# harvardinformatics/IMCoalHMM

Hardware: AMD Instinct MI355X
Metric: alignment columns/sec (forward pass), 20-state isolation HMM (higher is better)
Workload: dtype f64

## Files before the change

imcoalhmm_amd/csrc/imcoal_fwd.hip:

```cpp
#include <hip/hip_runtime.h>

#include <algorithm>
#include <array>
#include <cerrno>
#include <climits>
#include <cmath>
#include <cstdint>
#include <cstdio>
#include <cstdlib>
#include <cstring>
#include <list>
#include <atomic>
#include <chrono>
#include <map>
#include <set>
#include <memory>
#include <mutex>
#include <condition_variable>
#include <string>
#include <vector>

#include <sys/stat.h>
#include <unistd.h>

// ... 5 lines not shown
#include "kernels_zip2.hpp"
#include "kernels_zip3.hpp"
#include "kernels_zip4.hpp"
#include "pair_dict.hpp"
#include "kernels_encode.hpp"
#include "kernels_train.hpp"
#include "kernels_ingest.hpp"
#include "kernels_align.hpp"
#include "plan_host.hpp"
#include "planner_host.hpp"
#include "model_host.hpp"
#include "kernels_model.hpp"
#include "../../include/imcoal_model.h"
#include "obs_io.hpp"
#include "fasta_io.hpp"

static_assert(sizeof(imc::Desc4) == sizeof(int4) && alignof(imc::Desc4) == alignof(int4), "descriptor entries are uploaded as int4");

namespace {

thread_local std::string g_err;
std::mutex g_mu;
std::condition_variable g_cv;

int fail(int code, const std::string &msg)
{
    g_err = msg;
    return code;
}

#define HIP_TRY(expr)                                                                                   \
    do {                                                                                                \
        hipError_t _e = (expr);                                                                         \
        if (_e != hipSuccess)                                                                           \
            return fail(_e == hipErrorOutOfMemory ? IMC_ERR_OOM : IMC_ERR_HIP,                          \
                        std::string(#expr) + ": " + hipGetErrorString(_e));                             \
    } while (0)

using imc::HYBRID_MAX_ALPHABET;
using imc::LDS_BUDGET;
using imc::Z2GRAN;
using imc::round_up;

constexpr size_t STAGE_KERNEL_MAX_BYTES = 1u << 20;

hipError_t dev_alloc(void **p, size_t bytes);
void dev_free(void *p);

struct DictDev : imc::TrainedDict {
    uint16_t *d_left = nullptr, *d_right = nullptr;
    uint16_t *d_order = nullptr;
    uint64_t trained_on = 0;
    pid_t pid = 0;
    DictDev(imc::TrainedDict t, uint64_t columns) : imc::TrainedDict(std::move(t)), trained_on(columns) {}
    ~DictDev()
    {
        if (pid == getpid()) { dev_free(d_left); dev_free(d_right); dev_free(d_order); }
    }
};

struct Ev3 { hipEvent_t a, b, c; };

struct Ctx {
    pid_t pid = 0;
    int device = -1;
    bool ready = false;
    hipStream_t stream = nullptr;
    int cus = 256;
    uint64_t next_obs_id = 1, next_dict_id = 1;
    size_t seg_override = 0;
    int compression = 1;
    int kernel_pref = 0;
    bool profile = false;
    bool rank1_handoff = true;
    int blocked_variant = 4;
    int wide_blocked = -1;
    int z4_stream = -1;
    bool table_pairs = true;
    int table_triples = -1;
    bool table_split = true;
    int table_split_max = -1;
    bool xcd_affine = true;
    int fuse_tail = 1;
    bool fuse_head = true;
    bool pack_table = true;
    int device_encode = -1;
    bool guard = false;
    bool use_graphs = false;
    std::vector<Ev3> events;
    std::map<int, std::shared_ptr<DictDev>> dicts;
    uint64_t last_plan[8] = {0, 0, 0, 0, 0, 0, 0, 0};
    uint64_t last_ingest[4] = {0, 0, 0, 0};
    int device_ingest = -1;
    int device_train = -1;
    uint64_t last_training[4] = {0, 0, 0, 0};
    uint64_t r1_checked = 0, r1_collapsed = 0;
    std::string last_kernels;
    std::vector<const void *> lds_opted;
} g;

void drop_plans();
void drop_plans_using(imc_obs *const *obs, size_t n);
void wait_all_idle(std::unique_lock<std::mutex> &lk);
void model_release();

int ensure_ctx()
{
    const pid_t me = getpid();
    if (g.ready && g.pid == me) return IMC_OK;
    if (g.ready && g.pid != me)
        return fail(IMC_ERR_HIP, "libimcoal_fwd was initialised in the parent process before fork(): fork the chain "
                                 "processes before the first imc_* call of the parent, or use the spawn start method");
    int n = 0;
    if (hipGetDeviceCount(&n) != hipSuccess || n <= 0)
        return fail(IMC_ERR_NODEVICE, "no HIP device available (libimcoal_fwd has no CPU fallback)");
    if (g.device < 0) {
        int cur = 0;
        if (hipGetDevice(&cur) != hipSuccess) cur = 0;
        g.device = cur;
    }
    if (g.device >= n) return fail(IMC_ERR_NODEVICE, "requested device index out of range");
    HIP_TRY(hipSetDevice(g.device));
    hipDeviceProp_t prop;
    HIP_TRY(hipGetDeviceProperties(&prop, g.device));
    if (std::strncmp(prop.gcnArchName, "gfx950", 6) != 0)
        return fail(IMC_ERR_NODEVICE, std::string("device is ") + prop.gcnArchName + ", this library is built for gfx950 only");
    g.cus = prop.multiProcessorCount > 0 ? prop.multiProcessorCount : 256;
    HIP_TRY(hipStreamCreateWithFlags(&g.stream, hipStreamNonBlocking));
    g.use_graphs = std::getenv("IMC_GRAPH") != nullptr;
    if (const char *gd = std::getenv("IMC_GUARD")) g.guard = std::atoi(gd) != 0;
    if (const char *bv = std::getenv("IMC_BLOCKED")) { const int v = std::atoi(bv); if (v >= 2 && v <= 5) g.blocked_variant = v; }
    if (const char *r1 = std::getenv("IMC_RANK1")) g.rank1_handoff = std::atoi(r1) != 0;
    if (const char *pt = std::getenv("IMC_PACK_TABLE")) g.pack_table = std::atoi(pt) != 0;
    if (const char *tp = std::getenv("IMC_TABLE_PAIRS")) g.table_pairs = std::atoi(tp) != 0;
    if (const char *fh = std::getenv("IMC_FUSE_HEAD")) g.fuse_head = std::atoi(fh) != 0;
    if (const char *ts = std::getenv("IMC_TABLE_SPLIT")) g.table_split = std::atoi(ts) != 0;
    if (const char *tm = std::getenv("IMC_TABLE_SPLIT_MAX")) g.table_split_max = std::max(0, std::atoi(tm));
    if (const char *tt = std::getenv("IMC_TABLE_TRIPLES")) g.table_triples = std::atoi(tt) != 0 ? 1 : 0;
    if (const char *ft = std::getenv("IMC_FUSE_TAIL")) g.fuse_tail = std::max(0, std::min(2, std::atoi(ft)));
    if (const char *xa = std::getenv("IMC_XCD_AFFINE")) g.xcd_affine = std::atoi(xa) != 0;
    if (const char *wb = std::getenv("IMC_WIDE_BLOCKED")) { const int v = std::atoi(wb); if (v >= -1 && v <= 1) g.wide_blocked = v; }
    if (g.device_encode < 0) {
        const char *de = std::getenv("IMC_DEVICE_ENCODE");
        g.device_encode = de && std::atoi(de) == 1 ? 1 : 0;
    }
    if (const char *zs = std::getenv("IMC_Z4_STREAM")) { const int v = std::atoi(zs); if (v >= -1 && v <= 1) g.z4_stream = v; }
    g.pid = me;
    g.ready = true;
    return IMC_OK;
}

struct GuardRec { hipDeviceptr_t va; size_t va_size; hipMemGenericAllocationHandle_t handle; hipDeviceptr_t map; size_t map_size; };
std::map<void *, GuardRec> &g_guard = *new std::map<void *, GuardRec>();

hipError_t dev_alloc(void **p, size_t bytes)
{
    bytes = std::max<size_t>(bytes, 16);
    if (!g.guard) return hipMalloc(p, bytes);
    hipMemAllocationProp prop{};
    prop.type = hipMemAllocationTypePinned;
    prop.location.type = hipMemLocationTypeDevice;
    prop.location.id = g.device;
    size_t gran = 0;
    hipError_t e = hipMemGetAllocationGranularity(&gran, &prop, hipMemAllocationGranularityMinimum);
    if (e != hipSuccess || gran == 0) return e != hipSuccess ? e : hipErrorUnknown;
    GuardRec r{};
    r.map_size = (bytes + gran - 1) / gran * gran;
    r.va_size = r.map_size + 2 * gran;
    e = hipMemAddressReserve(&r.va, r.va_size, gran, nullptr, 0);
    if (e != hipSuccess) return e;
    e = hipMemCreate(&r.handle, r.map_size, &prop, 0);
    if (e != hipSuccess) { (void)hipMemAddressFree(r.va, r.va_size); return e; }
    r.map = (hipDeviceptr_t)((char *)r.va + gran);
    e = hipMemMap(r.map, r.map_size, 0, r.handle, 0);
    if (e == hipSuccess) {
        hipMemAccessDesc ad{};
        ad.location = prop.location;
        ad.flags = hipMemAccessFlagsProtReadWrite;
        e = hipMemSetAccess(r.map, r.map_size, &ad, 1);
        if (e != hipSuccess) (void)hipMemUnmap(r.map, r.map_size);
    }
    if (e != hipSuccess) { (void)hipMemRelease(r.handle); (void)hipMemAddressFree(r.va, r.va_size); return e; }
    void *user = (char *)r.map + (r.map_size - (bytes + 15) / 16 * 16);
    g_guard[user] = r;
    *p = user;
    return hipSuccess;
}

void dev_free(void *p)
{
    if (!p) return;
    auto it = g_guard.find(p);
    if (it == g_guard.end()) { (void)hipFree(p); return; }
    (void)hipDeviceSynchronize();
    (void)hipMemUnmap(it->second.map, it->second.map_size);
    (void)hipMemRelease(it->second.handle);
    g_guard.erase(it);
}

template <class T>
class DevBuf {
    T *p_ = nullptr;

public:
    DevBuf() = default;
    DevBuf(const DevBuf &) = delete;
    DevBuf &operator=(const DevBuf &) = delete;
    DevBuf(DevBuf &&o) noexcept : p_(o.p_) { o.p_ = nullptr; }
    DevBuf &operator=(DevBuf &&o) noexcept
    {
        if (this != &o) { reset(); p_ = o.p_; o.p_ = nullptr; }
        return *this;
    }
    ~DevBuf() { reset(); }
    hipError_t alloc(size_t bytes)
    {
        reset();
        return dev_alloc((void **)&p_, bytes);
    }
    void reset()
    {
        dev_free(p_);
        p_ = nullptr;
// ... 1192 lines not shown
}

int recompress_alphabet(int nsym, std::vector<imc_obs *> &obs, bool on_device)
{
    std::sort(obs.begin(), obs.end(), [](const imc_obs *x, const imc_obs *y) { return x->id < y->id; });
    obs.erase(std::unique(obs.begin(), obs.end()), obs.end());
    const bool wide_raw = nsym > imc::kByteAlphabet;
    const size_t unit = wide_raw ? sizeof(imc::tok_t) : 1;
    PhaseTimer tm;
    size_t total = 0;
    for (imc_obs *o : obs) total += o->L;
    if (total < imc::TrainLimits().train_min) return IMC_OK;
    const size_t share = imc::recompress_share(obs.size(), wide_raw);
    std::vector<std::vector<uint8_t>> raw(obs.size());
    bool train_on_device = false;
    size_t copied = 0;
    {
        std::lock_guard<std::mutex> lk(g_mu);
        train_on_device = device_train_mode() == 1;
        bool same = obs[0]->dict != nullptr;
        for (imc_obs *o : obs) same = same && o->dict == obs[0]->dict;
        if (same && obs[0]->dict->trained_on >= total) return IMC_OK;
        HIP_TRY(hipSetDevice(g.device));
        for (size_t k = 0; k < obs.size() && !(train_on_device && on_device); ++k) {
            raw[k].resize((on_device ? std::min(obs[k]->L, share) : obs[k]->L) * unit);
            HIP_TRY(hipMemcpy(raw[k].data(), obs[k]->d_sym, raw[k].size(), hipMemcpyDeviceToHost));
            copied += raw[k].size();
        }
    }
    std::vector<uint8_t> sample;
    if (!train_on_device) sample = imc::recompress_sample(raw, share, unit);
    tm.mark();
    std::shared_ptr<DictDev> nd;
    if (train_on_device) {
        std::vector<TrainPiece> pieces;
        size_t sample_len = 0;
        for (imc_obs *o : obs) {
            pieces.push_back({o->d_sym, (int)unit, std::min(o->L, share)});
            sample_len += pieces.back().n;
        }
        std::lock_guard<std::mutex> lk(g_mu);
        HIP_TRY(hipSetDevice(g.device));
        if (int rc = device_train(pieces.data(), pieces.size(), nsym, sample_len, total, &nd)) return rc;
    } else {
        imc::TrainStats st;
        nd = make_dictionary(symbols_in(sample, wide_raw), nsym, total, &st);
        std::vector<uint8_t>().swap(sample);
        std::lock_guard<std::mutex> lk(g_mu);
        note_training(0, st);
    }
    tm.mark();
    std::vector<imc::EncodedLevels> enc(obs.size());
    const bool zipped = nd->dict.alphabet > nsym;
    if (zipped && !on_device)
        for (size_t k = 0; k < obs.size(); ++k) {
            const HostSymbols sym = symbols_in(raw[k], wide_raw);
            imc::encode_levels(nd->dict, sym.bytes, sym.wide, obs[k]->L, enc[k]);
            std::vector<uint8_t>().swap(raw[k]);
        }
    tm.mark();
    std::unique_lock<std::mutex> lk(g_mu);
    wait_all_idle(lk);
    HIP_TRY(hipSetDevice(g.device));
    HIP_TRY(hipDeviceSynchronize());
    drop_plans_using(obs.data(), obs.size());
    if (!zipped) return IMC_OK;
    if (int rc = publish_dictionary(nsym, nd)) return rc;
    if (on_device) {
        for (imc_obs *o : obs) release_tokens(o);
        if (int rc = device_encode(nd, obs.data(), obs.size())) return rc;
    } else
        for (size_t k = 0; k < obs.size(); ++k) {
            release_tokens(obs[k]);
            if (int rc = install_encoding(obs[k], nd, enc[k])) return rc;
        }
    tm.mark();
    if (PhaseTimer::enabled())
        std::fprintf(stderr, "[imc host] recompress %zu chunks, %zu columns: copy back %.1f ms, train %.1f ms, encode %.1f ms, install %.1f ms (%s encoder, %s trainer, %zu symbol bytes to the host)\n",
                     obs.size(), total, tm.ms(0), tm.ms(1), tm.ms(2), tm.ms(3), on_device ? "device" : "host", train_on_device ? "device" : "host", copied);
    return IMC_OK;
}


using ChainFn = void (*)(const ChainDesc *, int, const uint32_t *, uint32_t, uint32_t, const double *, const int *,
                         const int *, uint32_t, double *, int *, double *, int);

struct KernelChoice : imc::KernelFacts {
    void (*plain)(PropArgs) = nullptr;
    void (*zip)(PropArgs) = nullptr;
    ChainFn chain = nullptr;
    void (*big_table_raw)(BigArgs) = nullptr;
    void (*big_table_level)(BigArgs, const uint16_t *, int) = nullptr;
    void (*big_prop)(BigArgs, const BigBlock *) = nullptr;
    int big_prop_waves = 0;
    void (*big_vec)(BigArgs, const BigBlock *, int, int) = nullptr;
    void (*big_vec_tail)(BigArgs, const BigBlock *, int, int) = nullptr;
    int big_vec_waves = 0;
    void (*zip2)(BigArgs) = nullptr;
    void (*zip3)(BigArgs) = nullptr;
    void (*zip4)(BigArgs) = nullptr;
    void (*zip4w)(BigArgs) = nullptr;
    void (*zip4s)(BigArgs) = nullptr, (*zip4sw)(BigArgs) = nullptr;
    void (*zip4_raw)(BigArgs) = nullptr;
    void (*zip4_level)(BigArgs, int, int) = nullptr;
    void (*zip4_level2)(BigArgs, const int4 *, int, int, const double *) = nullptr;
    void (*zip4_level2_first)(BigArgs, const int4 *, int, int, const double *) = nullptr;
    void (*zip4_level2_split)(BigArgs, const int4 *, int, int, const double *) = nullptr;
    void (*zip4_level2_split_first)(BigArgs, const int4 *, int, int, const double *) = nullptr;
    void (*zip4_level3)(BigArgs, const int4 *, int, int, const double *) = nullptr;
    void (*zip4_level3_first)(BigArgs, const int4 *, int, int, const double *) = nullptr;
    size_t (*zip4_level3_lds)(size_t) = nullptr;
    bool chain_self_emax = false;
    void note_kernels()
    {
        has_zip2 = zip2 != nullptr; has_zip3 = zip3 != nullptr; has_zip4 = zip4 != nullptr; has_zip4s = zip4s != nullptr;
        has_level2 = zip4_level2 != nullptr;
    }
};

template <int R, int G, int MW>
KernelChoice make_kc()
{
    constexpr int NP = R * G;
    KernelChoice k;
    k.R = R; k.G = G; k.NP = NP; k.VPW = 64 / G; k.minw = MW;
    k.zwaves = ZWAVES;
    k.z4_waves = Z2WAVES;
    k.plain = k_propagate<R, G, MW>;
    k.zip = k_zpropagate<R, G>;
    k.zip_lds = &ZipGeom<R, G>::lds_bytes;
    k.chain = k_chain<NP, (NP <= 12 ? 6 : NP <= 24 ? 4 : NP <= 32 ? 3 : NP <= 64 ? 2 : 1)>;
    k.chain_self_emax = true;
    if constexpr (NP % 4 == 0 && NP <= 24) {
        k.zip2 = k_zpropagate2<NP / 4>;
        k.zip2_lds = &Zip2Geom<NP / 4>::lds_bytes;
        k.zip3 = k_zpropagate3<NP / 4>;
        k.zip3_lds = &Zip3Geom<NP / 4>::lds_bytes;
        k.tok_doubles = Zip3Geom<NP / 4>::TOK;
        if constexpr (NP <= 24) {
            k.zip4 = k_zpropagate4<NP / 4, false, true>;
            k.zip4w = k_zpropagate4<NP / 4, true, true>;
            k.zip4s = k_zpropagate4<NP / 4, false, false>;
            k.zip4sw = k_zpropagate4<NP / 4, true, false>;
            k.zip4_raw = k_z4_raw<NP / 4>;
            k.zip4_level = k_z4_level<NP / 4>;
            k.zip4_level2 = k_z4_level2<NP / 4, false>;
            k.zip4_level2_first = k_z4_level2<NP / 4, true>;
            k.zip4_level2_split = k_z4_level2<NP / 4, false, Z4_SPLIT_WAVES>;
            k.zip4_level2_split_first = k_z4_level2<NP / 4, true, Z4_SPLIT_WAVES_FIRST>;
            k.zip4_level3 = k_z4_level3<NP / 4, false>;
            k.zip4_level3_first = k_z4_level3<NP / 4, true>;
            k.zip4_level3_lds = &Z4L3Geom<NP / 4>::lds_bytes;
            k.zip4_lds = &Zip4Geom<NP / 4>::lds_bytes;
            k.zip4_max_hot = &Zip4Geom<NP / 4>::max_hot;
        }
    }
    if constexpr (NP == 28 || NP == 32) {
        k.tok_doubles = Zip3Geom<NP / 4>::TOK;
        k.zip4s = k_zpropagate4<NP / 4, false, false>;
        k.zip4sw = k_zpropagate4<NP / 4, true, false>;
        k.zip4_raw = k_z4_raw<NP / 4>;
        k.zip4_level = k_z4_level<NP / 4>;
        k.zip4_lds = &Zip4Geom<NP / 4>::lds_bytes;
        k.z4_waves = Zip4Shape<NP / 4>::WAVES;
        k.wide_blocked = true;
    }
    k.note_kernels();
    return k;
}

template <int NT, int NSLAB>
KernelChoice make_big()
{
    constexpr bool dealt = NT > 4 && NT % 4 != 0;
    KernelChoice k;
    k.G = NT; k.NP = 16 * NT;
    k.z4_waves = Z2WAVES;
    k.chain = k_chain<16 * NT, 0>;
    k.big_table_raw = k_big_table_raw<NT>;
    k.big_table_level = k_big_table_level<NT>;
    k.big_prop = k_big_propagate<NT, NSLAB>;
    if constexpr (dealt) k.big_prop = k_big_propagate_s<NT, NSLAB>;
    k.big_prop_waves = dealt ? BS_WAVES : NT;
    k.big_vec = k_big_vector<NT, false>;
    k.big_vec_tail = k_big_vector<NT, true>;
    k.big_vec_waves = BigVec<NT>::WAVES;
    k.big_nslab = NSLAB;
    k.big_lds = BigSlab<NT, NSLAB>::bytes;
    return k;
}

KernelChoice kChoices[] = {
    make_kc<4, 1, 2>(), make_kc<4, 2, 2>(), make_kc<4, 3, 2>(), make_kc<4, 4, 2>(), make_kc<4, 5, 2>(),
    make_kc<3, 8, 2>(), make_kc<2, 14, 2>(), make_kc<2, 16, 2>(), make_kc<2, 20, 1>(), make_kc<1, 48, 1>(),
    make_kc<1, 56, 1>(), make_kc<1, 64, 1>(),
    make_big<6, 1>(), make_big<7, 1>(), make_big<8, 2>(), make_big<9, 3>(), make_big<10, 2>(), make_big<12, 3>(), make_big<14, 7>(),
    make_big<16, 8>(),
};
constexpr int IMC_MAX_N = 256;

KernelChoice kMidChoices[] = {make_big<2, 1>(), make_big<3, 1>(), make_big<4, 1>()};

KernelChoice *choose_kernel(int N, bool prefer_gemm)
{
    if (prefer_gemm && N > 24 && N <= 64)
        for (auto &k : kMidChoices)
            if (k.NP >= N) return &k;
    for (auto &k : kChoices)
        if (k.NP >= N) return &k;
    return nullptr;
}


struct Group {
    using Kind = imc::GroupKind;
    Kind kind = Kind::ColumnVector;
    bool is_chain() const { return kind == Kind::GemmChain || kind == Kind::MatVecChain; }
    bool is_blocked() const { return kind == Kind::BlockedLds || kind == Kind::BlockedGlobal; }
    bool global_table() const { return kind == Kind::BlockedGlobal; }

    bool tokens = false;
    int level = -1, A = 0;
    std::shared_ptr<DictDev> dict;
    std::vector<int> chunks;
    uint32_t vec_begin = 0, n_vecs = 0;
    size_t seglen = 0;
    double model_us = 0.0, model_tab_us = 0.0;
    uint64_t vsteps = 0;
    uint64_t stream_len = 0;
    DevBuf<double> d_Ctab;
    DevBuf<int> d_cex;

    struct Chain {
        std::vector<uint32_t> seg_ids, seg_out;
        std::vector<BigBlock> big_blocks;
        DevBuf<BigBlock> d_big_blocks;
        std::vector<std::pair<int, int>> table_runs;
        DevBuf<double> d_Cpack;
        bool rank1 = false;
        std::vector<int> checkpoints;
        std::vector<BigBlock> tail_blocks;
        std::vector<std::pair<uint32_t, uint32_t>> r1_segs;
        DevBuf<BigBlock> d_tail_blocks;
        DevBuf<int> d_r1flag, d_r1at;
        DevBuf<double> d_r1u, d_r1alpha;
    } chain;

    struct Blocked {
        std::vector<Z2Block> blocks;
        DevBuf<Z2Block> d_blocks;
        DevBuf<uint16_t> d_tab_order;
        DevBuf<int> d_tab_lvl;
        std::vector<int> tab_lvl;
        int tab_nlvl = 0;
        DevBuf<int4> d_tab_desc;
        DevBuf<int4> d_tab_desc2;
        std::vector<std::pair<int, int>> tab2;
        DevBuf<int4> d_tab_desc3;
        std::vector<std::pair<int, int>> tab3;
        bool wide_tokens = false;
        bool stream_table = false;
// ... 170 lines not shown
        chunk_unit.assign(n_chunks + 1, 0);
        for (int f = 0; f < n_chunks; ++f) chunk_unit[f + 1] = chunk_unit[f] + (uint32_t)chunk_units[f].size();
        unit_vec0.assign(chunk_unit[n_chunks], 0);
        unit_first.assign(chunk_unit[n_chunks], 0);
        for (Group &gr : p->groups) {
            gr.vec_begin = (uint32_t)vecs.size();
            for (int f : gr.chunks) {
                gr.stream_len += gr.tokens ? chunks[f]->ntok[gr.level] : chunks[f]->L;
                for (size_t u = 0; u < chunk_units[f].size(); ++u) {
                    const uint32_t sid = chunk_units[f][u].first, ns = chunk_units[f][u].second;
                    const uint32_t uid = chunk_unit[f] + (uint32_t)u;
                    const bool fst = seg_first[sid] != 0;
                    unit_first[uid] = fst;
                    unit_vec0[uid] = (uint32_t)vecs.size();
                    const int nv = fst ? 1 : N;
                    for (int c = 0; c < nv; ++c) vecs.push_back(VecDesc{sid, (uint32_t)c});
                    if (gr.is_chain()) { gr.chain.seg_ids.push_back(sid); gr.chain.seg_out.push_back(unit_vec0[uid]); }
                    if (gr.is_blocked()) {
                        std::vector<Z2Block> &blocks = gr.blk.blocks;
                        const bool whole = mfma() && fst && ns == 1 && chunk_units[f].size() == 1;
                        if (whole && !blocks.empty() && blocks.back().first == 2 && blocks.back().n < (uint32_t)kc->z4_slots() &&
                            blocks.back().seg0 + blocks.back().n == sid && blocks.back().out_vec0 + blocks.back().n == unit_vec0[uid])
                            ++blocks.back().n;
                        else
                            blocks.push_back(Z2Block{sid, ns, unit_vec0[uid], whole ? 2u : fst ? 1u : 0u});
                    }
                    for (uint32_t q2 = 0; q2 < ns; ++q2)
                        gr.vsteps += (uint64_t)((seg_first[sid + q2] && !gr.is_blocked()) ? 1 : N) * segs[sid + q2].len;
                }
            }
            gr.n_vecs = (uint32_t)vecs.size() - gr.vec_begin;
        }
        if (p->groups.size() == 1 && p->groups[0].is_blocked() && mfma() && !op_mode && n_chunks > 0) {
            Group::Blocked &bl = p->groups[0].blk;
            bool ok = true;
            size_t most = 0;
            for (int f = 0; f < n_chunks; ++f) {
                ok = ok && !chunk_units[f].empty() && chunk_units[f].size() <= (size_t)kc->z4_slots();
                most = std::max(most, chunk_units[f].size());
            }
            if (ok) {
                for (int f : p->groups[0].chunks)
                    for (size_t u = 0; u < chunk_units[f].size(); ++u)
                        bl.tails.push_back(Z2Tail{(uint32_t)f, (uint32_t)u, (uint32_t)chunk_units[f].size(), 0u});
                bl.tail_stride = (int)most;
                if (bl.tails.size() != bl.blocks.size()) bl.tails.clear();
                else
                    for (Z2Block &bk : bl.blocks)
                        if (bk.first == 2) bk.first = 1;
            }
        }
        if (vecs.size() >= (size_t)UINT32_MAX / 2) return fail(IMC_ERR_ARG, "too many vectors in one call");
        p->n_segs = (uint32_t)segs.size();
        p->n_vecs = (uint32_t)vecs.size();
        p->pstride = round_up((size_t)kc->NP + (size_t)kc->NP * kc->NP + (size_t)S * kc->NP, 2);

        return IMC_OK;
    }

    void make_hierarchy()
    {
        hl.assign(1, HostLevel());
        hl[0].chunk_seg = chunk_unit; hl[0].vec0 = unit_vec0; hl[0].first = unit_first; hl[0].n_vecs = p->n_vecs;
        for (;;) {
            const HostLevel &cur = hl.back();
            uint32_t kmax = 0;
            for (int f = 0; f < n_chunks; ++f) kmax = std::max(kmax, cur.chunk_seg[f + 1] - cur.chunk_seg[f]);
            if (kmax <= 1 && hl.size() > 1) break;
            if (kmax == 0) break;
            const uint32_t gsz = kmax <= 16 ? kmax : std::max<uint32_t>(12, (uint32_t)std::ceil(std::cbrt((double)kmax)));
            p->chain_steps += gsz;
            HostLevel nx;
            nx.chunk_seg.assign(n_chunks + 1, 0);
            nx.n_vecs = 0;
            for (int f = 0; f < n_chunks; ++f) {
                nx.chunk_seg[f] = (uint32_t)nx.vec0.size();
                const uint32_t s0 = cur.chunk_seg[f], s1 = cur.chunk_seg[f + 1];
                for (uint32_t rb = s0; rb < s1; rb += gsz) {
                    const uint32_t re = std::min(rb + gsz, s1);
                    const bool fst = rb == s0 && !op_mode;
                    nx.vec0.push_back(nx.n_vecs);
                    nx.first.push_back(fst);
                    const int nvv = fst ? 1 : N;
                    for (int c = 0; c < nvv; ++c) nx.chains.push_back(ChainDesc{rb, re, (uint32_t)c, nx.n_vecs + c, fst ? 1u : 0u, 0u});
                    nx.n_vecs += nvv;
                }
            }
            nx.chunk_seg[n_chunks] = (uint32_t)nx.vec0.size();
            const bool done = kmax <= gsz;
            hl.push_back(std::move(nx));
            if (done) break;
        }
        final_vec.assign(std::max(n_chunks, 1), -1);
        bool all_from_chains = hl.size() > 1 && !op_mode && n_chunks > 0;
        for (int f = 0; f < n_chunks; ++f) {
            const HostLevel &last = hl.back();
            if (last.chunk_seg[f + 1] > last.chunk_seg[f]) final_vec[f] = (int32_t)last.vec0[last.chunk_seg[f]];
            else all_from_chains = false;
        }
        p->finish_fused = false;
        if (all_from_chains) {
            HostLevel &last = hl.back();
            std::vector<char> seen((size_t)n_chunks, 0);
            for (ChainDesc &cd : last.chains)
                for (int f = 0; f < n_chunks; ++f)
                    if (cd.first && final_vec[f] == (int32_t)cd.out_vec) { cd.chunk1 = (uint32_t)f + 1; seen[f] = 1; }
            p->finish_fused = std::all_of(seen.begin(), seen.end(), [](char c) { return c != 0; });
            if (!p->finish_fused)
                for (ChainDesc &cd : last.chains) cd.chunk1 = 0;
        }

    }

    int upload(Plan **out)
    {
        while (g_plans.size() >= MAX_PLANS) {
            auto victim = g_plans.end();
            for (auto it = g_plans.begin(); it != g_plans.end(); ++it)
                if (!(*it)->busy) victim = it;
            if (victim == g_plans.end()) break;
            g_plans.erase(victim);
        }

        Plan *q = p.get();
        DevUpload u;
        u.put(q->d_segs, segs);
        u.put(q->d_vecs, vecs);
        u.put(q->d_final_vec, final_vec);
        q->levels.resize(hl.size());
        for (size_t l = 0; l < hl.size(); ++l) {
            Level &lv = q->levels[l];
            lv.n_segs = (uint32_t)hl[l].vec0.size();
            lv.n_vecs = hl[l].n_vecs;
            lv.n_chains = (uint32_t)hl[l].chains.size();
            const size_t nv = std::max<size_t>(lv.n_vecs, 1), ns = std::max<size_t>(lv.n_segs, 1);
            u.put(lv.d_vec0, hl[l].vec0);
            u.put(lv.d_first, hl[l].first);
            u.put(lv.d_chains, hl[l].chains);
            u.zeroed(lv.d_P, (size_t)B * nv * kc->NP * 8);
            u.zeroed(lv.d_EX, (size_t)B * nv * 4);
            u.zeroed(lv.d_EMAX, (size_t)B * ns * 4);
        }
        for (Group &gr : q->groups) {
            Group::Blocked &bl = gr.blk;
            Group::Chain &ch = gr.chain;
            if (gr.is_blocked()) u.put(bl.d_blocks, bl.blocks);
            if (!bl.tails.empty()) {
                const size_t slots = (size_t)B * n_chunks * bl.tail_stride;
                u.put(bl.d_tails, bl.tails);
                u.alloc(bl.d_tailX, slots * kc->tok_doubles * 8);
                u.alloc(bl.d_tailE, slots * 128);
                u.zeroed(bl.d_tail_arrive, (size_t)B * n_chunks * 4);
            }
            if (gr.global_table()) {
                std::vector<uint64_t> cnt((size_t)gr.A, 0);
                for (int f : gr.chunks)
                    for (size_t z = 0; z < chunks[f]->tok_count[gr.level].size() && z < cnt.size(); ++z) cnt[z] += chunks[f]->tok_count[gr.level][z];
                const std::vector<uint16_t> ids = imc::hot_order(cnt);
                const double tables = (double)B * (gr.A + 1) * kc->tok_doubles * 8.0;
                bl.stream_table = wide || imc::z4_streamed(opt, tables, B);
                bl.n_hot = bl.stream_table ? 0 : std::min(gr.A, kc->zip4_max_hot(gr.A, LDS_BUDGET));
                bl.hot.assign(ids.begin(), ids.begin() + bl.n_hot);
                bl.phases = imc::xcd_phases(B, (int)bl.blocks.size());
                u.put(bl.d_hot, bl.hot);
                u.alloc(gr.d_Ctab, (size_t)B * (gr.A + 1) * kc->tok_doubles * 8);
                u.alloc(gr.d_cex, (size_t)B * (gr.A + 1) * 4 + 16);
            }
// ... 413 lines not shown
        }
    return IMC_OK;
}

int Launch::zip4(const Group &gr)
{
    BigArgs ba = blocked_args(gr);
    if (int rc = z4_table(gr, ba)) return rc;
    void (*scan)(BigArgs) = gr.blk.stream_table ? (gr.blk.wide_tokens ? kc->zip4sw : kc->zip4s) : (gr.blk.wide_tokens ? kc->zip4w : kc->zip4);
    if (int rc = allow_lds_budget(scan)) return rc;
    if (int rc = mark_a()) return rc;
    dim3 scan_grid(ba.n_group_segs, (unsigned)B);
    if (g.xcd_affine && B > 1) {
        const imc::PhaseTable &t = gr.blk.phases;
        ba.n_phases = t.n_phases;
        for (int k = 0; k < t.n_phases; ++k) { ba.ph_begin[k] = t.ph_begin[k]; ba.ph_first[k] = t.ph_first[k]; ba.ph_sets[k] = t.ph_sets[k]; }
        scan_grid = dim3((unsigned)t.grid);
    }
    hipLaunchKernelGGL(scan, scan_grid, dim3(kc->z4_waves * 64), kc->zip4_lds(gr.A, gr.blk.n_hot), stream, ba);
    note(std::string("k_zpropagate4<") + std::to_string(kc->NP / 4) + (gr.blk.wide_tokens ? ",16" : "") + (gr.blk.stream_table ? ",streamed>" : ">") + stream_tag(gr));
    account(gr);
    HIP_TRY(hipGetLastError());
    return IMC_OK;
}

int Launch::zip32(const Group &gr)
{
    BigArgs ba = blocked_args(gr);
    const bool v3 = kc->use3(g.blocked_variant);
    void (*scan)(BigArgs) = v3 ? kc->zip3 : kc->zip2;
    if (int rc = allow_lds_budget(scan)) return rc;
    size_t lds3 = kc->blocked_lds(gr.A, g.blocked_variant);
    if (direct_params) { ba.params_src = p->h_params_dev[p->slot]; lds3 = ((lds3 + 15) & ~(size_t)15) + p->pstride * 8; }
    hipLaunchKernelGGL(scan, dim3(ba.n_group_segs, (unsigned)p->B), dim3(Z2WAVES * 64), lds3, stream, ba);
    note(std::string(v3 ? "k_zpropagate3<" : "k_zpropagate2<") + std::to_string(kc->NP / 4) + ">" + stream_tag(gr));
    account(gr);
    HIP_TRY(hipGetLastError());
    return IMC_OK;
}


int Launch::zpropagate(const Group &gr)
{
    const size_t lds = kc->zip_lds(gr.A);
    if (int rc = allow_lds_budget(kc->zip)) return rc;
    const uint32_t vpb = (uint32_t)(ZWAVES * kc->VPW);
    dim3 grid((gr.n_vecs + vpb - 1) / vpb, (unsigned)p->B);
    hipLaunchKernelGGL(kc->zip, grid, dim3(ZWAVES * 64), lds, stream, prop_args(p, gr));
    note("k_zpropagate<" + std::to_string(kc->R) + "," + std::to_string(kc->G) + ">" + stream_tag(gr));
    account(gr);
    HIP_TRY(hipGetLastError());
    return IMC_OK;
}

int Launch::propagate(const Group &gr)
{
    const uint32_t vpb = (uint32_t)(WPB * kc->VPW);
    dim3 grid((gr.n_vecs + vpb - 1) / vpb, (unsigned)p->B);
    const size_t lds = ((size_t)WPB * kc->VPW * kc->NP + (size_t)p->S * kc->NP) * 8;
    if (lds > LDS_BUDGET) return fail(IMC_ERR_ARG, "emission table (S x N) too large for LDS");
    if (lds > 48 * 1024)
        if (int rc = allow_lds_budget(kc->plain)) return rc;
    hipLaunchKernelGGL(kc->plain, grid, dim3(WPB * 64), lds, stream, prop_args(p, gr));
    note("k_propagate<" + std::to_string(kc->R) + "," + std::to_string(kc->G) + ">" + stream_tag(gr));
    account(gr);
    HIP_TRY(hipGetLastError());
    return IMC_OK;
}


int Launch::stitch() const
{
    const int N = p->N, NP = kc->NP;
    for (size_t l = 0; l + 1 < p->levels.size(); ++l) {
        const Level &in = p->levels[l], &ot = p->levels[l + 1];
        if (!in.n_segs || !ot.n_chains) continue;
        if (!kc->chain_self_emax) {
            hipLaunchKernelGGL(k_emax, dim3((in.n_segs + 255) / 256, (unsigned)B), dim3(256), 0, stream,
                               in.d_vec0.get(), in.d_first.get(), in.n_segs, in.n_vecs, N, in.d_EX.get(), in.d_EMAX.get());
            HIP_TRY(hipGetLastError());
        }
        const int threads = (int)round_up((size_t)NP, 64);
        const bool last_level = l + 2 == p->levels.size();
        hipLaunchKernelGGL(kc->chain, dim3(ot.n_chains, (unsigned)B), dim3(threads), 0, stream,
                           ot.d_chains.get(), N, in.d_vec0.get(), in.n_segs, in.n_vecs, in.d_P.get(), in.d_EX.get(), in.d_EMAX.get(),
                           ot.n_vecs, ot.d_P.get(), ot.d_EX.get(), (last_level && p->finish_fused) ? out : (double *)nullptr, p->n_chunks);
        HIP_TRY(hipGetLastError());
    }
    if (p->n_chunks && !p->finish_fused) {
        const Level &last = p->levels.back();
        hipLaunchKernelGGL(k_finish, dim3((p->n_chunks + 63) / 64, (unsigned)B), dim3(64), 0, stream,
                           p->d_final_vec.get(), p->n_chunks, N, NP, last.n_vecs, last.d_P.get(), last.d_EX.get(), out);
        HIP_TRY(hipGetLastError());
    }
    return IMC_OK;
}

int enqueue(Plan *p, hipStream_t stream, double *out, bool allow_tail = true)
{
    hipStreamCaptureStatus cap = hipStreamCaptureStatusNone;
    (void)hipStreamIsCapturing(stream, &cap);
    if (cap == hipStreamCaptureStatusNone && p->have_last && p->last_stream != stream)
        HIP_TRY(hipStreamWaitEvent(stream, p->ev_params[p->last_slot], 0));
    Launch L{p, stream, out, allow_tail};
    if (int rc = L.fetch_params()) return rc;

    uint64_t *lp = p->lp;
    lp[0] = p->n_segs; lp[1] = p->n_vecs; lp[2] = lp[3] = lp[4] = lp[5] = lp[6] = lp[7] = 0;
    L.prof = g.profile && p->n_vecs;
    if (L.prof) { HIP_TRY(hipEventCreate(&L.ev.a)); HIP_TRY(hipEventCreate(&L.ev.b)); HIP_TRY(hipEventCreate(&L.ev.c)); }
    p->kernels.clear();
    for (const Group &gr : p->groups) {
        if (!gr.n_vecs) continue;
        if (!gr.global_table())
            if (int rc = L.mark_a()) return rc;
        int rc = IMC_OK;
        switch (gr.kind) {
        case Group::Kind::ColumnVector: rc = L.propagate(gr); break;
        case Group::Kind::TokenVector: rc = L.zpropagate(gr); break;
        case Group::Kind::BlockedLds: rc = L.zip32(gr); break;
        case Group::Kind::BlockedGlobal: rc = L.zip4(gr); break;
        case Group::Kind::GemmChain: rc = L.gemm_chain(gr); break;
        case Group::Kind::MatVecChain: rc = L.matvec_chain(gr); break;
        }
        if (rc) return rc;
    }
    if (int rc = L.mark_a()) return rc;
    if (L.prof) HIP_TRY(hipEventRecord(L.ev.b, stream));
    if (L.split_used) L.note("table-split");
    if (L.tail_used) L.note("fused-tail");
    if (!L.tail_used)
        if (int rc = L.stitch()) return rc;
    if (L.prof) {
        HIP_TRY(hipEventRecord(L.ev.c, stream));
        g.events.push_back(L.ev);
    }
    if (cap == hipStreamCaptureStatusNone) {
        HIP_TRY(hipEventRecord(p->ev_params[p->slot], stream));
        p->ev_used[p->slot] = true;
        p->last_stream = stream;
        p->last_slot = p->slot;
        p->have_last = true;
    }
    return IMC_OK;
}

void collect_rank1_stats(Plan *p)
{
    g.r1_checked = g.r1_collapsed = 0;
    for (Group &gr : p->groups) {
        if (!gr.chain.rank1 || gr.chain.r1_segs.empty() || gr.chain.checkpoints.empty()) continue;
        std::vector<int> flags((size_t)p->B * p->n_segs);
        if (hipMemcpy(flags.data(), gr.chain.d_r1flag.get(), flags.size() * 4, hipMemcpyDeviceToHost) != hipSuccess) continue;
        for (int b = 0; b < p->B; ++b)
            for (const auto &sl : gr.chain.r1_segs) {
                if ((int)sl.second <= gr.chain.checkpoints[0]) continue;
                ++g.r1_checked;
                g.r1_collapsed += flags[(size_t)b * p->n_segs + sl.first] ? 1 : 0;
            }
        if (getenv("IMC_DEBUG_R1")) {
            std::vector<int> at((size_t)p->B * p->n_segs);
            if (hipMemcpy(at.data(), gr.chain.d_r1at.get(), at.size() * 4, hipMemcpyDeviceToHost) != hipSuccess) continue;
            std::map<int, int> hist;
            for (const auto &sl : gr.chain.r1_segs) hist[flags[sl.first] ? at[sl.first] : -1]++;
            fprintf(stderr, "[imc] rank-one hand-off: segment length %zu tokens, checkpoints", (size_t)gr.seglen);
            for (int c : gr.chain.checkpoints) fprintf(stderr, " %d", c);
            fprintf(stderr, "\n[imc]   certified at (tokens: segments)");
            for (auto &kv : hist) fprintf(stderr, " %d:%d", kv.first, kv.second);
// ... 1062 lines not shown
```

imcoalhmm_amd/csrc/kernels_stitch.hpp:

```cpp
#pragma once
#include "kernels_plain.hpp"

struct ChainDesc {
    uint32_t seg_begin, seg_end;
    uint32_t c;
    uint32_t out_vec;
    uint32_t first;
    uint32_t chunk1;
};

__global__ void k_emax(const uint32_t *seg_vec0, const uint8_t *seg_first, uint32_t n_segs, uint32_t n_vecs, int N,
                       const int *EX, int *EMAX)
{
    const uint32_t s = blockIdx.x * blockDim.x + threadIdx.x;
    const int b = blockIdx.y;
    if (s >= n_segs) return;
    const int *e = EX + (size_t)b * n_vecs + seg_vec0[s];
    int m = e[0];
    if (!seg_first[s])
        for (int c = 1; c < N; ++c) m = max(m, e[c]);
    EMAX[(size_t)b * n_segs + s] = m;
}

template <int NP, int D>
__global__ __launch_bounds__(((NP + 63) / 64) * 64) void k_chain(
    const ChainDesc *chains, int N,
    const uint32_t *in_vec0, uint32_t in_n_segs, uint32_t in_n_vecs, const double *Pin, const int *EXin, const int *EMin,
    uint32_t out_n_vecs, double *Pout, int *EXout, double *fin_out, int n_chunks)
{
    __shared__ __attribute__((aligned(16))) double w[2][NP];
    constexpr bool ONE_WAVE = NP <= 64;
    auto sync = [&]() { if (ONE_WAVE) wave_fence(); else __syncthreads(); };
    const ChainDesc cd = chains[blockIdx.x];
    const int b = blockIdx.y, i = threadIdx.x;
    const double *Pb = Pin + (size_t)b * in_n_vecs * NP;
    const int *EXb = EXin + (size_t)b * in_n_vecs;
    const int *EMb = EMin + (size_t)b * in_n_segs;
    const bool mine = i < N;
    const int ii = mine ? i : 0;

    double a;
    int etot;
    uint32_t k0 = cd.seg_begin;
    if (cd.first) {
        const uint32_t v = in_vec0[k0];
        a = mine ? Pb[(size_t)v * NP + i] : 0.0;
        etot = EXb[v];
        ++k0;
    } else {
        a = (i == (int)cd.c) ? 1.0 : 0.0;
        etot = 0;
    }
    const int nsteps = (int)cd.seg_end - (int)k0;
    const uint32_t vbase = nsteps > 0 ? in_vec0[k0] : 0u;

    if constexpr (D == 0) {
        int buf = 0;
        for (int t = 0; t < nsteps; ++t) {
            const size_t v0 = (size_t)vbase + (size_t)t * N;
            const int em = EMb[k0 + t];
            if (mine) w[buf][i] = ldexp(a, EXb[v0 + ii] - em);
            else if (i < NP) w[buf][i] = 0.0;
            sync();
            const double2 *row = reinterpret_cast<const double2 *>(Pb + (v0 + ii) * NP);
            const double2 *wv = reinterpret_cast<const double2 *>(&w[buf][0]);
            double acc0 = 0.0, acc1 = 0.0, s0 = 0.0, s1 = 0.0;
#pragma unroll 4
            for (int m = 0; m < NP / 2; ++m) {
                const double2 wc = wv[m], pc = row[m];
                acc0 = fma(pc.x, wc.x, acc0);
                acc1 = fma(pc.y, wc.y, acc1);
                s0 += wc.x;
                s1 += wc.y;
            }
            const double sm = s0 + s1;
            int e = 0;
            (void)frexp(sm, &e);
            e = (sm > 0.0 && sm < INFINITY) ? e : 0;
            a = mine ? ldexp(acc0 + acc1, -e) : 0.0;
            etot += em + e;
            buf ^= 1;
        }
    } else {
    double2 pk[D > 0 ? D : 1][NP / 2];
    int exr[D > 0 ? D : 1];
    auto fetch = [&](int t, int slot) {
        const size_t v0 = (size_t)vbase + (size_t)t * N;
        exr[slot] = EXb[v0 + ii];
        const double2 *row = reinterpret_cast<const double2 *>(Pb + (v0 + ii) * NP);
#pragma unroll
        for (int m = 0; m < NP / 2; ++m) pk[slot][m] = row[m];
    };
#pragma unroll
    for (int s = 0; s < D; ++s)
        if (s < nsteps) fetch(s, s);
    int buf = 0;
    for (int t0 = 0; t0 < nsteps; t0 += D) {
#pragma unroll
        for (int s = 0; s < D; ++s) {
            const int t = t0 + s;
            if (t < nsteps) {
                const int em = wave_max_i32_dpp(exr[s]);
                if (mine) w[buf][i] = ldexp(a, exr[s] - em);
                else if (i < NP) w[buf][i] = 0.0;
                double2 cur[NP / 2];
#pragma unroll
                for (int m = 0; m < NP / 2; ++m) cur[m] = pk[s][m];
                if (t + D < nsteps) fetch(t + D, s);
                sync();
                double acc0 = 0.0, acc1 = 0.0, s0 = 0.0, s1 = 0.0;
                const double2 *wv = reinterpret_cast<const double2 *>(&w[buf][0]);
#pragma unroll
                for (int m = 0; m < NP / 2; ++m) {
                    const double2 wc = wv[m];
                    acc0 = fma(cur[m].x, wc.x, acc0);
                    acc1 = fma(cur[m].y, wc.y, acc1);
                    s0 += wc.x;
                    s1 += wc.y;
                }
                const double sm = s0 + s1;
                int e = 0;
                (void)frexp(sm, &e);
                e = (sm > 0.0 && sm < INFINITY) ? e : 0;
                a = mine ? ldexp(acc0 + acc1, -e) : 0.0;
                etot += em + e;
                buf ^= 1;
            }
        }
    }
    }
    sync();
    if (i < NP) w[0][i] = mine ? a : 0.0;
    sync();
    double tot = 0.0;
    for (int c = 0; c < N; ++c) tot += w[0][c];
    int e = 0;
    (void)frexp(tot, &e);
    e = (tot > 0.0 && tot < INFINITY) ? e : 0;
    const size_t gv = (size_t)b * out_n_vecs + cd.out_vec;
    if (mine) {
        double *dst = cd.first ? Pout + gv * NP + i : Pout + (gv - cd.c) * NP + (size_t)i * NP + cd.c;
        *dst = ldexp(a, -e);
    }
    if (i == 0) {
        EXout[gv] = etot + e;
        if (fin_out && cd.chunk1)
            fin_out[(size_t)b * n_chunks + (cd.chunk1 - 1)] = (double)(etot + e) * 0.693147180559945309417232121458 + log(ldexp(tot, -e));
    }
}

__global__ void k_finish(const int32_t *final_vec, int n_chunks, int N, int NP, uint32_t n_vecs, const double *P,
                         const int *EX, double *out)
{
    const int f = blockIdx.x * blockDim.x + threadIdx.x;
    const int b = blockIdx.y;
    if (f >= n_chunks) return;
    const int32_t v = final_vec[f];
    double r = 0.0;
    if (v >= 0) {
        const double *p = P + ((size_t)b * n_vecs + v) * NP;
        double tot = 0.0;
        for (int c = 0; c < N; ++c) tot += p[c];
        r = (double)EX[(size_t)b * n_vecs + v] * 0.693147180559945309417232121458 + log(tot);
    }
    out[(size_t)b * n_chunks + f] = r;
}

__global__ void k_export(const int32_t *final_vec, int n_chunks, int N, int NP, uint32_t n_vecs, const double *P,
                         const int *EX, int op, double *out_state, int *out_exp)
{
    const int f = blockIdx.x, b = blockIdx.y;
    const int32_t v = final_vec[f];
    if (v < 0) return;
    const double *src = P + ((size_t)b * n_vecs + v) * NP;
    const int *ex = EX + (size_t)b * n_vecs + v;
    if (op) {
        double *dst = out_state + ((size_t)b * n_chunks + f) * N * N;
        int *de = out_exp + ((size_t)b * n_chunks + f) * N;
        for (int idx = threadIdx.x; idx < N * N; idx += blockDim.x) {
            const int i = idx / N, c = idx - i * N;
            dst[idx] = src[(size_t)i * NP + c];
        }
        for (int c = threadIdx.x; c < N; c += blockDim.x) de[c] = ex[c];
    } else {
        double *dst = out_state + ((size_t)b * n_chunks + f) * N;
        for (int i = threadIdx.x; i < N; i += blockDim.x) dst[i] = src[i];
        if (threadIdx.x == 0) out_exp[(size_t)b * n_chunks + f] = ex[0];
    }
}

__global__ void k_stage_params(const double2 *__restrict__ src, double2 *__restrict__ dst, unsigned n2)
{
    const unsigned i = blockIdx.x * blockDim.x + threadIdx.x;
    if (i < n2) dst[i] = src[i];
}

__global__ void k_sum_chunks(const double *per_chunk, int n_chunks, int B, double *partial)
{
    const int b = blockIdx.x * blockDim.x + threadIdx.x;
    if (b >= B) return;
    double t = 0.0;
    for (int f = 0; f < n_chunks; ++f) t += per_chunk[(size_t)b * n_chunks + f];
    partial[b] = t;
}
```

Measured before the change: 393.3 billion.

## Broadcast chain state via DPP/permlane instead of LDS, precompute chain vector bases

Result: no change. 397.7 billion, median of 6 (+1.1%).

```diff
diff --git a/imcoalhmm_amd/csrc/imcoal_fwd.hip b/imcoalhmm_amd/csrc/imcoal_fwd.hip
--- a/imcoalhmm_amd/csrc/imcoal_fwd.hip
+++ b/imcoalhmm_amd/csrc/imcoal_fwd.hip
@@ -111,6 +111,7 @@
     int table_split_max = -1;
     bool xcd_affine = true;
     int fuse_tail = 1;
+    bool chain_lds = false;
     bool fuse_head = true;
     bool pack_table = true;
     int device_encode = -1;
@@ -168,6 +169,7 @@
     if (const char *tt = std::getenv("IMC_TABLE_TRIPLES")) g.table_triples = std::atoi(tt) != 0 ? 1 : 0;
     if (const char *ft = std::getenv("IMC_FUSE_TAIL")) g.fuse_tail = std::max(0, std::min(2, std::atoi(ft)));
     if (const char *xa = std::getenv("IMC_XCD_AFFINE")) g.xcd_affine = std::atoi(xa) != 0;
+    if (const char *cl = std::getenv("IMC_CHAIN_LDS")) g.chain_lds = std::atoi(cl) != 0;
     if (const char *wb = std::getenv("IMC_WIDE_BLOCKED")) { const int v = std::atoi(wb); if (v >= -1 && v <= 1) g.wide_blocked = v; }
     if (g.device_encode < 0) {
         const char *de = std::getenv("IMC_DEVICE_ENCODE");
@@ -1526,13 +1528,14 @@
 }
 
 
-using ChainFn = void (*)(const ChainDesc *, int, const uint32_t *, uint32_t, uint32_t, const double *, const int *,
+using ChainFn = void (*)(const ChainDesc *, int, uint32_t, uint32_t, const double *, const int *,
                          const int *, uint32_t, double *, int *, double *, int);
 
 struct KernelChoice : imc::KernelFacts {
     void (*plain)(PropArgs) = nullptr;
     void (*zip)(PropArgs) = nullptr;
     ChainFn chain = nullptr;
+    ChainFn chain_lds = nullptr;
     void (*big_table_raw)(BigArgs) = nullptr;
     void (*big_table_level)(BigArgs, const uint16_t *, int) = nullptr;
     void (*big_prop)(BigArgs, const BigBlock *) = nullptr;
@@ -1573,7 +1576,9 @@
     k.plain = k_propagate<R, G, MW>;
     k.zip = k_zpropagate<R, G>;
     k.zip_lds = &ZipGeom<R, G>::lds_bytes;
-    k.chain = k_chain<NP, (NP <= 12 ? 6 : NP <= 24 ? 4 : NP <= 32 ? 3 : NP <= 64 ? 2 : 1)>;
+    constexpr int CHAIN_D = NP <= 12 ? 6 : NP <= 24 ? 4 : NP <= 32 ? 3 : NP <= 64 ? 2 : 1;
+    k.chain = k_chain<NP, CHAIN_D, CHAIN_STEP>;
+    k.chain_lds = k_chain<NP, CHAIN_D, CHAIN_LDS>;
     k.chain_self_emax = true;
     if constexpr (NP % 4 == 0 && NP <= 24) {
         k.zip2 = k_zpropagate2<NP / 4>;
@@ -1620,7 +1625,7 @@
     KernelChoice k;
     k.G = NT; k.NP = 16 * NT;
     k.z4_waves = Z2WAVES;
-    k.chain = k_chain<16 * NT, 0>;
+    k.chain = k.chain_lds = k_chain<16 * NT, 0>;
     k.big_table_raw = k_big_table_raw<NT>;
     k.big_table_level = k_big_table_level<NT>;
     k.big_prop = k_big_propagate<NT, NSLAB>;
@@ -1957,7 +1962,10 @@
                     nx.vec0.push_back(nx.n_vecs);
                     nx.first.push_back(fst);
                     const int nvv = fst ? 1 : N;
-                    for (int c = 0; c < nvv; ++c) nx.chains.push_back(ChainDesc{rb, re, (uint32_t)c, nx.n_vecs + c, fst ? 1u : 0u, 0u});
+                    const uint32_t op0 = rb + (fst ? 1u : 0u);
+                    const uint32_t vec_first = fst ? cur.vec0[rb] : 0u, vbase = op0 < re ? cur.vec0[op0] : 0u;
+                    for (int c = 0; c < nvv; ++c)
+                        nx.chains.push_back(ChainDesc{rb, re, (uint32_t)c, nx.n_vecs + c, fst ? 1u : 0u, 0u, vec_first, vbase});
                     nx.n_vecs += nvv;
                 }
             }
@@ -2537,8 +2545,8 @@
         }
         const int threads = (int)round_up((size_t)NP, 64);
         const bool last_level = l + 2 == p->levels.size();
-        hipLaunchKernelGGL(kc->chain, dim3(ot.n_chains, (unsigned)B), dim3(threads), 0, stream,
-                           ot.d_chains.get(), N, in.d_vec0.get(), in.n_segs, in.n_vecs, in.d_P.get(), in.d_EX.get(), in.d_EMAX.get(),
+        hipLaunchKernelGGL(g.chain_lds ? kc->chain_lds : kc->chain, dim3(ot.n_chains, (unsigned)B), dim3(threads), 0, stream,
+                           ot.d_chains.get(), N, in.n_segs, in.n_vecs, in.d_P.get(), in.d_EX.get(), in.d_EMAX.get(),
                            ot.n_vecs, ot.d_P.get(), ot.d_EX.get(), (last_level && p->finish_fused) ? out : (double *)nullptr, p->n_chunks);
         HIP_TRY(hipGetLastError());
     }
diff --git a/imcoalhmm_amd/csrc/kernels_stitch.hpp b/imcoalhmm_amd/csrc/kernels_stitch.hpp
--- a/imcoalhmm_amd/csrc/kernels_stitch.hpp
+++ b/imcoalhmm_amd/csrc/kernels_stitch.hpp
@@ -1,5 +1,6 @@
 #pragma once
 #include "kernels_plain.hpp"
+#include <utility>
 
 struct ChainDesc {
     uint32_t seg_begin, seg_end;
@@ -7,7 +8,44 @@
     uint32_t out_vec;
     uint32_t first;
     uint32_t chunk1;
+    uint32_t vec_first;
+    uint32_t vbase;
 };
+
+enum ChainForm { CHAIN_LDS = 0, CHAIN_LANE = 1, CHAIN_DPP = 2 };
+static constexpr int CHAIN_STEP = CHAIN_DPP;
+
+template <int... M, class F>
+__device__ __forceinline__ void static_for(std::integer_sequence<int, M...>, F &&f) { (f(std::integral_constant<int, M>()), ...); }
+
+template <int M>
+__device__ __forceinline__ double lane_bcast_f64(double x)
+{
+    const int lo = __builtin_amdgcn_readlane(__double2loint(x), M), hi = __builtin_amdgcn_readlane(__double2hiint(x), M);
+    return __hiloint2double(hi, lo);
+}
+
+template <int NR>
+__device__ __forceinline__ void rows_to_all(double x, double (&rows)[NR])
+{
+    static_assert(NR >= 1 && NR <= 4, "a wavefront has four rows");
+    const unsigned lo = (unsigned)__double2loint(x), hi = (unsigned)__double2hiint(x);
+    if constexpr (NR == 1) {
+        rows[0] = x;
+    } else if constexpr (NR == 2) {
+        const auto l = __builtin_amdgcn_permlane16_swap(lo, lo, false, false), h = __builtin_amdgcn_permlane16_swap(hi, hi, false, false);
+        rows[0] = __hiloint2double((int)h[0], (int)l[0]);
+        rows[1] = __hiloint2double((int)h[1], (int)l[1]);
+    } else {
+        const auto l = __builtin_amdgcn_permlane32_swap(lo, lo, false, false), h = __builtin_amdgcn_permlane32_swap(hi, hi, false, false);
+        const auto l0 = __builtin_amdgcn_permlane16_swap(l[0], l[0], false, false), h0 = __builtin_amdgcn_permlane16_swap(h[0], h[0], false, false);
+        const auto l1 = __builtin_amdgcn_permlane16_swap(l[1], l[1], false, false), h1 = __builtin_amdgcn_permlane16_swap(h[1], h[1], false, false);
+        rows[0] = __hiloint2double((int)h0[0], (int)l0[0]);
+        rows[1] = __hiloint2double((int)h0[1], (int)l0[1]);
+        rows[2] = __hiloint2double((int)h1[0], (int)l1[0]);
+        if constexpr (NR == 4) rows[3] = __hiloint2double((int)h1[1], (int)l1[1]);
+    }
+}
 
 __global__ void k_emax(const uint32_t *seg_vec0, const uint8_t *seg_first, uint32_t n_segs, uint32_t n_vecs, int N,
                        const int *EX, int *EMAX)
@@ -22,12 +60,14 @@
     EMAX[(size_t)b * n_segs + s] = m;
 }
 
-template <int NP, int D>
+template <int NP, int D, int FORM = CHAIN_LDS>
 __global__ __launch_bounds__(((NP + 63) / 64) * 64) void k_chain(
     const ChainDesc *chains, int N,
-    const uint32_t *in_vec0, uint32_t in_n_segs, uint32_t in_n_vecs, const double *Pin, const int *EXin, const int *EMin,
+    uint32_t in_n_segs, uint32_t in_n_vecs, const double *Pin, const int *EXin, const int *EMin,
     uint32_t out_n_vecs, double *Pout, int *EXout, double *fin_out, int n_chunks)
 {
+    static_assert(FORM == CHAIN_LDS || (D > 0 && NP <= 64), "the register forms are for one wavefront");
+    constexpr int NR = (NP + 15) / 16;
     __shared__ __attribute__((aligned(16))) double w[2][NP];
     constexpr bool ONE_WAVE = NP <= 64;
     auto sync = [&]() { if (ONE_WAVE) wave_fence(); else __syncthreads(); };
@@ -43,7 +83,7 @@
     int etot;
     uint32_t k0 = cd.seg_begin;
     if (cd.first) {
-        const uint32_t v = in_vec0[k0];
+        const uint32_t v = cd.vec_first;
         a = mine ? Pb[(size_t)v * NP + i] : 0.0;
         etot = EXb[v];
         ++k0;
@@ -52,7 +92,7 @@
         etot = 0;
     }
     const int nsteps = (int)cd.seg_end - (int)k0;
-    const uint32_t vbase = nsteps > 0 ? in_vec0[k0] : 0u;
+    const uint32_t vbase = cd.vbase;
 
     if constexpr (D == 0) {
         int buf = 0;
@@ -83,7 +123,7 @@
         }
     } else {
     double2 pk[D > 0 ? D : 1][NP / 2];
-    int exr[D > 0 ? D : 1];
+    int exr[D > 0 ? D : 1] = {};
     auto fetch = [&](int t, int slot) {
         const size_t v0 = (size_t)vbase + (size_t)t * N;
         exr[slot] = EXb[v0 + ii];
@@ -94,46 +134,89 @@
 #pragma unroll
     for (int s = 0; s < D; ++s)
         if (s < nsteps) fetch(s, s);
+    int em = 0, sh = 0;
+    if (nsteps > 0) {
+        em = wave_max_i32_dpp(exr[0]);
+        sh = exr[0] - em;
+    }
     int buf = 0;
     for (int t0 = 0; t0 < nsteps; t0 += D) {
 #pragma unroll
         for (int s = 0; s < D; ++s) {
             const int t = t0 + s;
             if (t < nsteps) {
-                const int em = wave_max_i32_dpp(exr[s]);
-                if (mine) w[buf][i] = ldexp(a, exr[s] - em);
-                else if (i < NP) w[buf][i] = 0.0;
+                const double wi = mine ? ldexp(a, sh) : 0.0;
+                const int em_t = em;
                 double2 cur[NP / 2];
 #pragma unroll
                 for (int m = 0; m < NP / 2; ++m) cur[m] = pk[s][m];
                 if (t + D < nsteps) fetch(t + D, s);
-                sync();
+                em = wave_max_i32_dpp(exr[(s + 1) % D]);
+                sh = exr[(s + 1) % D] - em;
                 double acc0 = 0.0, acc1 = 0.0, s0 = 0.0, s1 = 0.0;
-                const double2 *wv = reinterpret_cast<const double2 *>(&w[buf][0]);
-#pragma unroll
-                for (int m = 0; m < NP / 2; ++m) {
-                    const double2 wc = wv[m];
-                    acc0 = fma(cur[m].x, wc.x, acc0);
-                    acc1 = fma(cur[m].y, wc.y, acc1);
-                    s0 += wc.x;
-                    s1 += wc.y;
+                auto column = [&](auto M, double wm) {
+                    constexpr int m = decltype(M)::value;
+                    if constexpr (m & 1) {
+                        acc1 = fma(cur[m / 2].y, wm, acc1);
+                        s1 += wm;
+                    } else {
+                        acc0 = fma(cur[m / 2].x, wm, acc0);
+                        s0 += wm;
+                    }
+                };
+                if constexpr (FORM == CHAIN_LDS) {
+                    if (i < NP) w[buf][i] = wi;
+                    sync();
+                    const double2 *wv = reinterpret_cast<const double2 *>(&w[buf][0]);
+#pragma unroll
+                    for (int m = 0; m < NP / 2; ++m) {
+                        const double2 wc = wv[m];
+                        acc0 = fma(cur[m].x, wc.x, acc0);
+                        acc1 = fma(cur[m].y, wc.y, acc1);
+                        s0 += wc.x;
+                        s1 += wc.y;
+                    }
+                    buf ^= 1;
+                } else if constexpr (FORM == CHAIN_LANE) {
+                    static_for(std::make_integer_sequence<int, NP>(), [&](auto M) { column(M, lane_bcast_f64<decltype(M)::value>(wi)); });
+                } else {
+                    double rows[NR];
+                    rows_to_all<NR>(wi, rows);
+                    static_for(std::make_integer_sequence<int, NP>(), [&](auto M) {
+                        constexpr int m = decltype(M)::value;
+                        column(M, __builtin_amdgcn_update_dpp(0.0, rows[m / 16], 0x150 + m % 16, 0xf, 0xf, true));
+                    });
                 }
                 const double sm = s0 + s1;
                 int e = 0;
                 (void)frexp(sm, &e);
                 e = (sm > 0.0 && sm < INFINITY) ? e : 0;
-                a = mine ? ldexp(acc0 + acc1, -e) : 0.0;
-                etot += em + e;
-                buf ^= 1;
+                a = ldexp(acc0 + acc1, -e);
+                etot += em_t + e;
             }
         }
     }
     }
-    sync();
-    if (i < NP) w[0][i] = mine ? a : 0.0;
-    sync();
     double tot = 0.0;
-    for (int c = 0; c < N; ++c) tot += w[0][c];
+    if constexpr (FORM == CHAIN_LDS) {
+        sync();
+        if (i < NP) w[0][i] = mine ? a : 0.0;
+        sync();
+        for (int c = 0; c < N; ++c) tot += w[0][c];
+    } else if constexpr (FORM == CHAIN_LANE) {
+        static_for(std::make_integer_sequence<int, NP>(), [&](auto M) {
+            const double am = lane_bcast_f64<decltype(M)::value>(a);
+            tot = decltype(M)::value < N ? tot + am : tot;
+        });
+    } else {
+        double rows[NR];
+        rows_to_all<NR>(a, rows);
+        static_for(std::make_integer_sequence<int, NP>(), [&](auto M) {
+            constexpr int m = decltype(M)::value;
+            const double am = __builtin_amdgcn_update_dpp(0.0, rows[m / 16], 0x150 + m % 16, 0xf, 0xf, true);
+            tot = m < N ? tot + am : tot;
+        });
+    }
     int e = 0;
     (void)frexp(tot, &e);
     e = (tot > 0.0 && tot < INFINITY) ? e : 0;
```
